# hzdr/PARIS

Measured on AMD Instinct MI355X. Metric: GVoxel-updates/s (voxels x projections / s), FDK hot path weight+filter+backproject, higher is better.
Workload: dtype f32

## Files before the change

include/paris_hip.h:

```cpp
#ifndef PARIS_HIP_H_
#define PARIS_HIP_H_

#include <stddef.h>
#include <stdint.h>

#ifdef __cplusplus
extern "C" {
#endif

#define PARIS_HIP_SUCCESS 0
#define PARIS_HIP_ERROR_INVALID_ARGUMENT 10001
#define PARIS_HIP_ERROR_NO_DEVICE 10002
#define PARIS_HIP_ERROR_UNSUPPORTED 10003

#define PARIS_HIP_CTX_DEFAULT 0u
#define PARIS_HIP_CTX_SYNCHRONOUS 1u
#define PARIS_HIP_CTX_LEGACY_STREAM 2u
#define PARIS_HIP_CTX_WARM 4u

typedef struct paris_detector_geometry {
    uint32_t n_row;
    uint32_t n_col;
    float l_px_row;
    float l_px_col;
// ... 194 lines not shown
                                uint32_t p_dim_y, uint32_t p_idx, float p_phi, float* d_v, uint32_t v_dim_x,
                                uint32_t v_dim_y, uint32_t v_dim_z, uint32_t v_offset,
                                const paris_detector_geometry* det_geo, const paris_volume_geometry* vol_geo,
                                int enable_angles, int enable_roi, const paris_region_of_interest* roi);

int paris_hip_forward_project(paris_hip_ctx* ctx, const float* d_v, uint32_t v_dim_x, uint32_t v_dim_y, uint32_t v_dim_z,
                              uint32_t v_offset, const paris_detector_geometry* det_geo, const paris_volume_geometry* vol_geo,
                              float* d_p, size_t p_pitch, size_t p_stride_bytes, uint32_t n_views, uint32_t p_dim_x,
                              uint32_t p_dim_y, const float* sin_phi, const float* cos_phi, float delta_s, float delta_t,
                              int accumulate);
int paris_hip_stage_forward_project(paris_hip_ctx* ctx, const float* d_v, uint32_t v_dim_x, uint32_t v_dim_y, uint32_t v_dim_z,
                                    uint32_t v_offset, const paris_detector_geometry* det_geo, const paris_volume_geometry* vol_geo,
                                    float* d_p, size_t p_pitch, uint32_t p_dim_x, uint32_t p_dim_y, uint32_t p_idx, float p_phi,
                                    int enable_angles, int accumulate);

const char* paris_hip_strerror(int status);
const char* paris_hip_version(void);
int paris_hip_has_experiments(void);
int paris_hip_last_backproject_ms(paris_hip_ctx* ctx, float* ms);
int paris_hip_backproject_timing_arm(paris_hip_ctx* ctx, uint32_t capacity);
int paris_hip_backproject_timing_collect(paris_hip_ctx* ctx, float* ms, uint32_t max_n, uint32_t* n_out);
int paris_hip_set_backproject_variant(paris_hip_ctx* ctx, int variant);
int paris_hip_set_backproject_tuning(paris_hip_ctx* ctx, int vx, int unroll, int tz, int lds_bytes);
int paris_hip_set_backproject_slice_shape(paris_hip_ctx* ctx, int waves, int row_groups);
int paris_hip_set_backproject_order(paris_hip_ctx* ctx, int order, int nontemporal);
int paris_hip_set_backproject_fast_division(paris_hip_ctx* ctx, int enable);
int paris_hip_set_backproject_vector_staging(paris_hip_ctx* ctx, int enable);
int paris_hip_fast_division_is_exact(paris_hip_ctx* ctx, float divisor, int* exact);
int paris_hip_lean_division_is_exact(paris_hip_ctx* ctx, float d_sd, float d_so, int* exact);
int paris_hip_lean_weighting_is_exact(paris_hip_ctx* ctx, float d_sd, float q_lo, float q_hi, int* exact);
int paris_hip_set_lean_validation(paris_hip_ctx* ctx, int enable);

#ifdef __cplusplus
}
#endif
#endif
```

paris_amd/_lib.py:

```python
import ctypes as C
import os

_HERE = os.path.dirname(os.path.abspath(__file__))
EXPERIMENTS_LIB_PATH = os.path.join(_HERE, "lib", "libparis_hip_experiments.so")
LIB_PATH = os.environ.get("PARIS_HIP_LIBRARY") or os.path.join(_HERE, "lib", "libparis_hip.so")

SUCCESS = 0
ERROR_INVALID_ARGUMENT = 10001
ERROR_NO_DEVICE = 10002
ERROR_UNSUPPORTED = 10003
CTX_DEFAULT = 0
CTX_SYNCHRONOUS = 1
CTX_LEGACY_STREAM = 2
CTX_WARM = 4
PIXEL_U8 = 1
PIXEL_U16 = 2
PIXEL_U32 = 3
PIXEL_F32 = 4


class DetectorGeometry(C.Structure):
    _fields_ = [("n_row", C.c_uint32), ("n_col", C.c_uint32),
                ("l_px_row", C.c_float), ("l_px_col", C.c_float),
                ("delta_s", C.c_float), ("delta_t", C.c_float),
# ... 115 lines not shown
    "paris_hip_short_scan_check": (C.c_int, [_P(DetectorGeometry), _P(ShortScan), _P(_f)]),
    "paris_hip_short_scan_weight_rows": (C.c_int, [_vp, _vp, _sz, _sz, _u32, _u32, _u32, _u32, _u32, _P(DetectorGeometry), _P(ShortScan),
                                                   _P(_f)]),
    "paris_hip_stage_short_scan_weight": (C.c_int, [_vp, _vp, _sz, _u32, _u32, _P(DetectorGeometry), _P(ShortScan), _u32, C.c_int,
                                                    _f]),
    "paris_hip_offset_detector_check": (C.c_int, [_P(DetectorGeometry), _P(_f)]),
    "paris_hip_offset_detector_weight_rows": (C.c_int, [_vp, _vp, _sz, _sz, _u32, _u32, _u32, _u32, _u32, _P(DetectorGeometry)]),
    "paris_hip_stage_offset_detector_weight": (C.c_int, [_vp, _vp, _sz, _u32, _u32, _P(DetectorGeometry)]),
    "paris_hip_stage_backproject": (C.c_int, [_vp, _vp, _sz, _u32, _u32, _u32, _f, _vp, _u32, _u32, _u32, _u32,
                                              _P(DetectorGeometry), _P(VolumeGeometry), C.c_int, C.c_int,
                                              _P(RegionOfInterest)]),
    "paris_hip_forward_project": (C.c_int, [_vp, _vp, _u32, _u32, _u32, _u32, _P(DetectorGeometry), _P(VolumeGeometry), _vp, _sz, _sz,
                                            _u32, _u32, _u32, _P(_f), _P(_f), _f, _f, C.c_int]),
    "paris_hip_stage_forward_project": (C.c_int, [_vp, _vp, _u32, _u32, _u32, _u32, _P(DetectorGeometry), _P(VolumeGeometry), _vp, _sz,
                                                  _u32, _u32, _u32, _f, C.c_int, C.c_int]),
    "paris_hip_strerror": (C.c_char_p, [C.c_int]),
    "paris_hip_version": (C.c_char_p, []),
    "paris_hip_last_backproject_ms": (C.c_int, [_vp, _P(_f)]),
    "paris_hip_backproject_timing_arm": (C.c_int, [_vp, _u32]),
    "paris_hip_backproject_timing_collect": (C.c_int, [_vp, _P(_f), _u32, _P(_u32)]),
    "paris_hip_set_backproject_variant": (C.c_int, [_vp, C.c_int]),
    "paris_hip_set_backproject_tuning": (C.c_int, [_vp, C.c_int, C.c_int, C.c_int, C.c_int]),
    "paris_hip_set_backproject_order": (C.c_int, [_vp, C.c_int, C.c_int]),
    "paris_hip_set_backproject_slice_shape": (C.c_int, [_vp, C.c_int, C.c_int]),
    "paris_hip_set_backproject_fast_division": (C.c_int, [_vp, C.c_int]),
    "paris_hip_set_backproject_vector_staging": (C.c_int, [_vp, C.c_int]),
    "paris_hip_fast_division_is_exact": (C.c_int, [_vp, _f, _P(C.c_int)]),
}

_lib = None


def load():
    global _lib
    if _lib is None:
        if not os.path.exists(LIB_PATH):
            raise ImportError(
                "paris_amd: %s not found -- build it with `python -c 'import __graft_entry__ as g; g.build()'` "
                "or `make -C paris_amd/csrc`; there is no CPU fallback" % LIB_PATH)
        if os.environ.get("PARIS_AMD_NO_TORCH") != "1":
            try:
                import torch
            except ImportError:
                pass
        lib = C.CDLL(LIB_PATH)
        for name, (res, args) in SIGNATURES.items():
# ... 23 lines not shown
```

paris_amd/backend.py:

```python
import ctypes as C

import numpy as np

from . import _lib
from ._lib import (DetectorGeometry, ParisHipError, RegionOfInterest, ShortScan, SubvolumeGeometry, SubvolumeInfo,
                   VolumeGeometry, check)

__all__ = ["DetectorGeometry", "VolumeGeometry", "SubvolumeGeometry", "RegionOfInterest", "SubvolumeInfo",
           "ParisHipError", "ShortScan", "Projection", "Volume", "FilterBuffer", "Backend", "get_devices", "set_device",
           "calculate_volume_geometry", "apply_roi", "filter_size", "load", "make_volume", "weight", "filter",
           "backproject", "forward_project", "short_scan_check", "offset_detector_check"]


class Projection:

    def __init__(self, buf, dim_x, dim_y, idx=0, phi=0.0, pitch=None, on_device=False, owner=None):
        self.buf = buf
        self.dim_x = dim_x
        self.dim_y = dim_y
        self.idx = idx
        self.phi = phi
        self.pitch = pitch if pitch is not None else dim_x * 4
        self.on_device = on_device
        self._owner = owner
# ... 332 lines not shown
              "paris_hip_forward_project")

    def last_backproject_ms(self):
        ms = C.c_float()
        check(self._L.paris_hip_last_backproject_ms(self._ctx, C.byref(ms)), "paris_hip_last_backproject_ms")
        return ms.value

    def backproject_timing_arm(self, capacity):
        check(self._L.paris_hip_backproject_timing_arm(self._ctx, capacity), "paris_hip_backproject_timing_arm")

    def backproject_timing_collect(self, max_n=65536):
        ms = (C.c_float * max_n)()
        n = C.c_uint32()
        check(self._L.paris_hip_backproject_timing_collect(self._ctx, ms, max_n, C.byref(n)),
              "paris_hip_backproject_timing_collect")
        return list(ms[:n.value])

    def set_backproject_variant(self, variant):
        check(self._L.paris_hip_set_backproject_variant(self._ctx, variant), "paris_hip_set_backproject_variant")

    def set_backproject_order(self, order=-1, nontemporal=-1):
        check(self._L.paris_hip_set_backproject_order(self._ctx, order, nontemporal), "paris_hip_set_backproject_order")

    def fast_division_is_exact(self, divisor):
        ok = C.c_int()
        check(self._L.paris_hip_fast_division_is_exact(self._ctx, divisor, C.byref(ok)), "paris_hip_fast_division_is_exact")
        return bool(ok.value)

    def set_backproject_vector_staging(self, enable=True):
        check(self._L.paris_hip_set_backproject_vector_staging(self._ctx, int(bool(enable))),
              "paris_hip_set_backproject_vector_staging")

    def set_backproject_fast_division(self, enable=True):
        check(self._L.paris_hip_set_backproject_fast_division(self._ctx, int(bool(enable))),
              "paris_hip_set_backproject_fast_division")

    def set_backproject_slice_shape(self, waves=0, row_groups=0):
        check(self._L.paris_hip_set_backproject_slice_shape(self._ctx, waves, row_groups),
              "paris_hip_set_backproject_slice_shape")

    def set_filter_window(self, window):
        check(self._L.paris_hip_set_filter_window(self._ctx, window), "paris_hip_set_filter_window")

    def set_filter_deferral(self, enable):
        check(self._L.paris_hip_set_filter_deferral(self._ctx, 2 if enable == 2 else int(bool(enable))), "paris_hip_set_filter_deferral")

# ... 165 lines not shown
```

paris_amd/csrc/backproject.hip:

```cpp
#include "bp_device.h"

#include <mutex>
#include <utility>

namespace
{
    __global__ void __launch_bounds__(256) fastdiv_validate_kernel(float c, float r, unsigned long long* mismatches)
    {
        const uint32_t t = blockIdx.x * 256u + threadIdx.x;
        unsigned int bad = 0;
        for(uint32_t i = 0; i < 256u; ++i)
        {
            const uint32_t bits = (i << 24) | t;
            const float x = __uint_as_float(bits);
            const float want = x / c - (1.f / 2.f);
            const float got = div_by_constant(x, c, r) - (1.f / 2.f);
            const bool same = __float_as_uint(want) == __float_as_uint(got);
            const bool both_nan = (want != want) && (got != got);
            const bool want_far = !(fabsf(want) <= 16777216.f);
            const bool got_far = !(fabsf(got) <= 16777216.f);
            if(!(same || both_nan || (want_far && got_far)))
                ++bad;
        }
        if(bad)
// ... 287 lines not shown
                       const paris_region_of_interest* roi, float sin_phi, float cos_phi, float delta_s, float delta_t,
                       BpParams& g, bool& fd, bool& skip)
{
    const size_t px = f16 ? sizeof(uint16_t) : sizeof(float);
    skip = false;
    if(int rc = paris_hip_bind(ctx))
        return rc;
    if(int rc = paris_hip_flush_pending_weight(ctx))
        return rc;
    if(d_p == nullptr || d_v == nullptr || det_geo == nullptr || vol_geo == nullptr || (enable_roi && roi == nullptr))
        return PARIS_HIP_ERROR_INVALID_ARGUMENT;
    if(p_dim_x == 0 || p_dim_y == 0 || p_pitch < static_cast<size_t>(p_dim_x) * px || p_pitch % px != 0)
        return PARIS_HIP_ERROR_INVALID_ARGUMENT;
    if(v_dim_x == 0 || v_dim_y == 0 || v_dim_z == 0)
    {
        skip = true;
        return PARIS_HIP_SUCCESS;
    }
    const uint64_t plane = static_cast<uint64_t>(v_dim_x) * v_dim_y;
    const uint32_t tz_auto = plane > (1ull << 20) ? (v_dim_z <= 256u ? 8u : TZ_DEFAULT) : (plane > (1ull << 18) ? 8u : TZ_DEFAULT);
    const uint32_t tz = ctx->bp_tz ? ctx->bp_tz : tz_auto;
    {
        const uint32_t tz_min = std::min(tz, 8u);
        const uint64_t ntx = (v_dim_x + 63u) / 64u, nty = (v_dim_y + 3u) / 4u, ntz = (v_dim_z + tz_min - 1u) / tz_min;
        const uint64_t zchunk = chunk_tiles(12u, tz_min, static_cast<uint32_t>(ntz), 64u);
        const uint64_t padded = std::max<uint64_t>(8ull * (8u * ((nty + 63u) / 64u)) * ntx * zchunk * ((ntz + zchunk - 1u) / zchunk),
                                                   8ull * ntx * nty * (ntz / 8u) + 8ull * 7u * 8u * ((nty + 63u) / 64u) * ntx);
        if(padded > 0x7fffff00ull)
            return PARIS_HIP_ERROR_UNSUPPORTED;
    }

    g = BpParams{};
    g.proj = d_p;
    g.proj_f16 = f16 ? 1u : 0u;
    g.vol = d_v;
    g.p_pitch = static_cast<uint32_t>(p_pitch / px);
    g.p_dim_x = p_dim_x;
    g.p_dim_y = p_dim_y;
    g.v_dim_x = v_dim_x;
    g.v_dim_y = v_dim_y;
    g.v_dim_z = v_dim_z;
    g.k_off = enable_roi ? roi->x1 : 0u;
    g.l_off = enable_roi ? roi->y1 : 0u;
    g.m_off = (enable_roi ? roi->z1 : 0u) + v_offset;
    g.x_base = centered_base(vol_geo->dim_x, vol_geo->l_vx_x);
    g.y_base = centered_base(vol_geo->dim_y, vol_geo->l_vx_y);
    g.z_base = centered_base(vol_geo->dim_z, vol_geo->l_vx_z);
    g.l_vx_x = vol_geo->l_vx_x;
    g.l_vx_y = vol_geo->l_vx_y;
    g.l_vx_z = vol_geo->l_vx_z;
// ... 18 lines not shown
        fd = fd && fd_x;
    }
    {
        const double x0 = g.x_base + static_cast<double>(g.k_off) * g.l_vx_x, x1 = g.x_base + (static_cast<double>(g.k_off) + v_dim_x - 1.0) * g.l_vx_x;
        const double y0 = g.y_base + static_cast<double>(g.l_off) * g.l_vx_y, y1 = g.y_base + (static_cast<double>(g.l_off) + v_dim_y - 1.0) * g.l_vx_y;
        const double reach = std::hypot(std::max(std::fabs(x0), std::fabs(x1)), std::max(std::fabs(y0), std::fabs(y1)));
        const double lo = std::ldexp(1.0, -40), hi = std::ldexp(1.0, 40);
        const bool ordinary = g.d_so >= lo && g.d_so <= hi && g.d_sd >= lo && g.d_sd <= hi;
        g.lean_div = (ctx->bp_lean_div != 0 && ordinary && std::isfinite(reach) && reach <= 0.9 * g.d_so) ? 1u : 0u;
        if(g.lean_div != 0u)
        {
            bool exact = false;
            if(int rc = paris_hip_lean_division_check(ctx, g.d_sd, g.d_so, &exact))
                return rc;
            g.lean_div = exact ? 1u : 0u;
        }
    }
    g.p_dim_x_f = static_cast<float>(p_dim_x);
    g.p_dim_y_f = static_cast<float>(p_dim_y);
    g.skip_invalid = (ctx->bp_skip_invalid != 0 && d_v != nullptr
                      && paris_hip_volume_is_clean(ctx, d_v, static_cast<size_t>(v_dim_x) * v_dim_y * v_dim_z * sizeof(float))) ? 1u : 0u;
    g.lds_floats = (ctx->bp_lds_bytes ? ctx->bp_lds_bytes : LDS_BYTES_DEFAULT) / sizeof(float);
    g.tz = tz;
    {
#ifdef PARIS_HIP_EXPERIMENTS
        static const int tile_nest = std::getenv("PARIS_TILE_NEST") ? std::atoi(std::getenv("PARIS_TILE_NEST")) : -1;
#else
        constexpr int tile_nest = -1;
#endif
        g.yfast = tile_nest >= 0 ? static_cast<uint32_t>(tile_nest) : (v_dim_z > 256u ? 2u : 0u);
    }
    g.order = ctx->bp_order >= 0 ? static_cast<uint32_t>(ctx->bp_order) : (plane > (1ull << 20) ? 15u : 18u);
    g.store_sc1 = volume_stream_policy(ctx, v_dim_x, v_dim_y, v_dim_z) == 2 ? 1u : 0u;
    g.stage_vec4 = (ctx->bp_stage_vec4 != 0 && g.p_pitch % 4u == 0 && reinterpret_cast<uintptr_t>(d_p) % (4u * px) == 0)
                       ? 1u : 0u;
    return PARIS_HIP_SUCCESS;
}

static int lane_width(const float* d_v, uint32_t v_dim_x)
{
    const uintptr_t addr = reinterpret_cast<uintptr_t>(d_v);
    if(v_dim_x % 4u == 0 && addr % 16u == 0)
        return 4;
    if(v_dim_x % 2u == 0 && addr % 8u == 0)
        return 2;
    return 1;
// ... 7 lines not shown
{
    BpParams g;
    bool fd = false, skip = false;
    if(int rc = fill_params(ctx, d_p, f16, p_pitch, p_dim_x, p_dim_y, d_v, v_dim_x, v_dim_y, v_dim_z, v_offset, det_geo, vol_geo,
                            enable_roi, roi, sin_phi, cos_phi, delta_s, delta_t, g, fd, skip))
        return rc;
    if(skip)
        return paris_hip_finish(ctx);

    const bool timed = !ctx->bp_start.empty();
    const size_t ev = timed ? static_cast<size_t>(ctx->bp_launches % ctx->bp_start.size()) : 0u;
    if(timed)
        PARIS_HIP_TRY(hipEventRecord(ctx->bp_start[ev], ctx->stream));
    if(ctx->bp_variant == 4 && !f16)
    {
        FusedParams fp{};
        fp.g = g;
        fp.n_proj = 1;
        fp.proj_tab[0] = d_p;
        fp.sin_phi[0] = sin_phi;
        fp.cos_phi[0] = cos_phi;
        const int width = lane_width(d_v, v_dim_x);
        const int vx = ctx->bp_vx == 4 && width == 4 ? 4 : (ctx->bp_vx == 1 || width < 2 ? 1 : 2);
        paris_hip_bp_launch_fused(&fp, vx, ctx->bp_tz == 8u ? 8 : (ctx->bp_tz == 32u ? 32 : 16), volume_stream_policy(ctx, v_dim_x, v_dim_y, v_dim_z) != 0, fd, ctx->stream);
    }
    else
    if(ctx->bp_variant == 1)
    {
        const dim3 grid((v_dim_x + 255u) / 256u, v_dim_y, v_dim_z);
        if(v_dim_y > 65535u || v_dim_z > 65535u)
            return PARIS_HIP_ERROR_UNSUPPORTED;
        hipLaunchKernelGGL(bp_gather_kernel, grid, dim3(256), 0, ctx->stream, g);
    }
    else
    {
        int vx = lane_width(d_v, v_dim_x);
        if(ctx->bp_vx && ctx->bp_vx < vx)
            vx = ctx->bp_vx;
        if(ctx->bp_vx == 0 && vx == 4 && ctx->bp_variant != 3 && ctx->bp_variant != 5)
        {
            const uint64_t tiles = static_cast<uint64_t>((v_dim_x + 63u) / 64u) * ((v_dim_y + 15u) / 16u) * ((v_dim_z + g.tz - 1u) / g.tz);
            if(tiles < 2048u)
                vx = 2;
        }
        const bool deep_big = g.tz == 16u && ctx->bp_tz == 0u && static_cast<uint64_t>(v_dim_x) * v_dim_y > (1ull << 20);
        if(deep_big && ctx->bp_unroll == 0 && ctx->bp_lds_bytes == 0u && vx == 4)
            g.lds_floats = 40u * 1024u / sizeof(float);
// ... 558 lines not shown
{
    if(int rc = paris_hip_flush_deferred(ctx))
        return rc;
    return batch_impl(ctx, d_p, true, p_pitch, p_stride_bytes, n_proj, p_dim_x, p_dim_y, d_v, v_dim_x, v_dim_y, v_dim_z, v_offset, det_geo,
                      vol_geo, enable_roi, roi, sin_phi, cos_phi, delta_s, delta_t);
}

static int batch_impl(paris_hip_ctx* ctx, const void* d_p, bool f16, size_t p_pitch, size_t p_stride_bytes, uint32_t n_proj, uint32_t p_dim_x,
                      uint32_t p_dim_y, float* d_v, uint32_t v_dim_x, uint32_t v_dim_y, uint32_t v_dim_z, uint32_t v_offset,
                      const paris_detector_geometry* det_geo, const paris_volume_geometry* vol_geo, int enable_roi,
                      const paris_region_of_interest* roi, const float* sin_phi, const float* cos_phi, float delta_s, float delta_t,
                      const void* const* ptrs)
{
    const size_t px = f16 ? sizeof(uint16_t) : sizeof(float);
    if(ctx == nullptr || sin_phi == nullptr || cos_phi == nullptr || (ptrs == nullptr && p_stride_bytes % px != 0))
        return PARIS_HIP_ERROR_INVALID_ARGUMENT;
    if(n_proj == 0)
        return paris_hip_finish(ctx);
    if(ptrs == nullptr && n_proj > 1 && p_stride_bytes < p_pitch * static_cast<size_t>(p_dim_y))
        return PARIS_HIP_ERROR_INVALID_ARGUMENT;
    const auto where = [&](uint32_t i) { return ptrs != nullptr ? static_cast<const char*>(ptrs[i]) : static_cast<const char*>(d_p) + static_cast<size_t>(i) * p_stride_bytes; };

    const int width = d_v != nullptr ? lane_width(d_v, v_dim_x) : 1;
    bool deep_box_fits = true;
    {
        const double d_so = std::fabs(static_cast<double>(det_geo->d_so)), d_sd = d_so + std::fabs(static_cast<double>(det_geo->d_od));
        const double mag = d_so > 0.0 ? d_sd / d_so : 1.0;
        const double rows = 32.0 * vol_geo->l_vx_z * mag / det_geo->l_px_col + 4.0 * std::max(vol_geo->l_vx_x, vol_geo->l_vx_y) * mag / det_geo->l_px_col + 8.0;
        const double cols = 64.0 * std::max(vol_geo->l_vx_x, vol_geo->l_vx_y) * mag / det_geo->l_px_row + 16.0;
        const double budget = ctx->bp_lds_bytes != 0u ? ctx->bp_lds_bytes : 32.0 * 1024.0;
        deep_box_fits = std::isfinite(rows) && std::isfinite(cols) && rows * std::max(132.0, cols) * sizeof(float) <= budget;
    }
    int fused_vx = ((v_dim_z <= 16u || !deep_box_fits) && width >= 2) ? 2 : 1;
    if(ctx->bp_vx == 4 && width == 4)
        fused_vx = 4;
    else if(ctx->bp_vx == 2 && width >= 2)
        fused_vx = 2;
    else if(ctx->bp_vx == 1)
        fused_vx = 1;
    int fused_tz = fused_vx == 1 ? ((v_dim_z <= 16u || !deep_box_fits) ? 16 : 32) : 16;
    if(ctx->bp_tz == 8u && fused_vx != 1)
        fused_tz = 8;
    else if(ctx->bp_tz == 16u)
        fused_tz = 16;
    else if(ctx->bp_tz == 32u && fused_vx == 1)
        fused_tz = 32;
    const bool fused_ok = n_proj > 1 && (ctx->bp_variant == 0 || ctx->bp_variant == 4) && d_v != nullptr;
    if(!fused_ok)
    {
        const unsigned saved = ctx->flags;
        ctx->flags &= ~PARIS_HIP_CTX_SYNCHRONOUS;
        int rc = PARIS_HIP_SUCCESS;
        for(uint32_t i = 0; i < n_proj && rc == PARIS_HIP_SUCCESS; ++i)
        {
            const char* p = where(i);
            rc = backproject_impl(ctx, p, f16, p_pitch, p_dim_x, p_dim_y, d_v, v_dim_x, v_dim_y, v_dim_z, v_offset, det_geo, vol_geo,
                                  enable_roi, roi, sin_phi[i], cos_phi[i], delta_s, delta_t);
        }
        ctx->flags = saved;
        if(rc != PARIS_HIP_SUCCESS)
            return rc;
        return paris_hip_finish(ctx);
    }

    const bool nt = volume_stream_policy(ctx, v_dim_x, v_dim_y, v_dim_z) != 0;
    for(uint32_t first = 0; first < n_proj; first += FUSED_MAX)
    {
        const uint32_t n = std::min<uint32_t>(FUSED_MAX, n_proj - first);
        FusedParams fp{};
        bool fd = false, skip = false;
        const char* p0 = where(first);
        if(int rc = fill_params(ctx, p0, f16, p_pitch, p_dim_x, p_dim_y, d_v, v_dim_x, v_dim_y, v_dim_z, v_offset, det_geo,
                                vol_geo, enable_roi, roi, sin_phi[first], cos_phi[first], delta_s, delta_t, fp.g, fd, skip))
            return rc;
        if(skip)
            break;
        fp.n_proj = n;
        if(ctx->bp_order < 0 && fp.g.order == 15u)
            fp.g.order = fused_vx == 1 ? 17u : (fused_vx == 2 ? 16u : 15u);
#ifdef PARIS_HIP_EXPERIMENTS
        static const bool x_fast = std::getenv("PARIS_FUSED_XFAST") != nullptr;
#else
        constexpr bool x_fast = false;
#endif
        fp.g.yfast = x_fast ? 0u : 1u;
        if(ctx->bp_lds_bytes == 0u)
            fp.g.lds_floats = 32u * 1024u / sizeof(float);
        for(uint32_t i = 0; i < n; ++i)
        {
            fp.sin_phi[i] = sin_phi[first + i];
            fp.cos_phi[i] = cos_phi[first + i];
            fp.proj_tab[i] = where(first + i);
            if(reinterpret_cast<uintptr_t>(fp.proj_tab[i]) % (4u * px) != 0)
                fp.g.stage_vec4 = 0u;
        }
        for(uint32_t i = n; i < FUSED_MAX; ++i)
            fp.proj_tab[i] = fp.proj_tab[0];
        const bool timed = !ctx->bp_start.empty();
        const size_t ev = timed ? static_cast<size_t>(ctx->bp_launches % ctx->bp_start.size()) : 0u;
        if(timed)
            PARIS_HIP_TRY(hipEventRecord(ctx->bp_start[ev], ctx->stream));
        paris_hip_bp_launch_fused(&fp, fused_vx, fused_tz, nt, fd, ctx->stream);
        if(timed)
            PARIS_HIP_TRY(hipEventRecord(ctx->bp_stop[ev], ctx->stream));
        ++ctx->bp_launches;
        for(uint32_t i = 0; i < n && !ctx->upload_targets.empty(); ++i)
            if(int rc = paris_hip_note_projection_use(ctx, where(first + i), p_pitch * p_dim_y))
                return rc;
    }
    return paris_hip_finish(ctx);
}

extern "C" int paris_hip_last_backproject_ms(paris_hip_ctx* ctx, float* ms)
{
    if(int rc = paris_hip_flush_deferred(ctx))
        return rc;
    if(ctx == nullptr || ms == nullptr || ctx->bp_launches == 0 || ctx->bp_start.empty())
        return PARIS_HIP_ERROR_INVALID_ARGUMENT;
    if(int rc = paris_hip_bind(ctx))
        return rc;
    const size_t ev = static_cast<size_t>((ctx->bp_launches - 1) % ctx->bp_start.size());
    PARIS_HIP_TRY(hipEventSynchronize(ctx->bp_stop[ev]));
    PARIS_HIP_TRY(hipEventElapsedTime(ms, ctx->bp_start[ev], ctx->bp_stop[ev]));
    return PARIS_HIP_SUCCESS;
}

extern "C" int paris_hip_set_backproject_variant(paris_hip_ctx* ctx, int variant)
{
    if(int rc = paris_hip_flush_deferred(ctx))
        return rc;
    if(ctx == nullptr || variant < 0 || variant > 5)
        return PARIS_HIP_ERROR_INVALID_ARGUMENT;
#ifndef PARIS_HIP_EXPERIMENTS
    if(variant == 3 || variant == 5)
        return PARIS_HIP_ERROR_UNSUPPORTED;
#endif
    ctx->bp_variant = variant;
    return PARIS_HIP_SUCCESS;
}

extern "C" int paris_hip_set_backproject_order(paris_hip_ctx* ctx, int order, int nontemporal)
{
    if(int rc = paris_hip_flush_deferred(ctx))
        return rc;
    if(ctx == nullptr || !(order == -1 || order == 0 || order == 1 || order == 5 || order == 8 || order == 9 || order == 12 || (order >= 14 && order <= 18)) || nontemporal < -1 || nontemporal > 2)
        return PARIS_HIP_ERROR_INVALID_ARGUMENT;
// ... 107 lines not shown
```

paris_amd/csrc/backproject_fused.hip:

```cpp
#define PARIS_BP_SINGLE_INSTRUCTION_FLOOR 1
#if (defined(PARIS_TIMING_ONLY_NO_BARRIERS) || defined(PARIS_TIMING_ONLY_STAGE_ONCE)) && !defined(PARIS_HIP_EXPERIMENTS)
#error "the timing-only switches compute WRONG results: they exist in the experiments build only (make EXPERIMENTS=1)"
#endif
#include "bp_device.h"

namespace
{
#ifndef PARIS_FUSED_PIPELINE
#define PARIS_FUSED_PIPELINE 1
#endif
#ifndef PARIS_FUSED_WAVES
#define PARIS_FUSED_WAVES 3
#endif
    constexpr int FIXED_STRIDE = 132;

    template <int VX, int TZ, bool NT, bool FD>
    __global__ void __launch_bounds__(256, PARIS_FUSED_WAVES + (VX == 2 ? 1 : VX == 1 ? (TZ == 32 ? 1 : 4) : 0) + (TZ == 8 ? 1 : 0)) bp_fused_kernel(const FusedParams fp)
    {
        extern __shared__ __attribute__((aligned(16))) float lds[];
        BpParams g = fp.g;
        using vec = typename vec_of<VX>::type;
        constexpr uint32_t XL = 64u / VX;
        constexpr uint32_t RW = VX;
        constexpr uint32_t TY = 4u * RW;

        const uint32_t tid = threadIdx.x;
        const uint32_t lane = tid & 63u;
        const uint32_t wave = tid >> 6;

        uint32_t bx, by, bz;
        if(!tile_of_block(g, blockIdx.x, bx, by, bz))
            return;
        const uint32_t k0 = bx * 64u;
        const uint32_t l0 = by * TY;
        const uint32_t m0 = bz * TZ;
        const uint32_t k1 = min(k0 + 63u, g.v_dim_x - 1u);
        const uint32_t l1 = min(l0 + TY - 1u, g.v_dim_y - 1u);
        const uint32_t m1 = min(m0 + TZ - 1u, g.v_dim_z - 1u);
        const uint32_t mcount = m1 - m0 + 1u;

        const uint32_t xq = lane % XL, yy = lane / XL;
        const uint32_t k = k0 + xq * VX;
        const uint32_t l = l0 + wave * RW + yy;
        const bool active = k < g.v_dim_x && l < g.v_dim_y;

        const size_t slice = static_cast<size_t>(g.v_dim_x) * g.v_dim_y;
        float* vp = g.vol + (static_cast<size_t>(m0) * g.v_dim_y + l) * g.v_dim_x + k;
        vec acc[TZ] = {};
#pragma unroll
        for(int z = 0; z < TZ; ++z)
            if(active && static_cast<uint32_t>(z) < mcount)
                acc[z] = load_voxels<VX, NT>(vp + z * slice);

        const float z_first = g.z_base + static_cast<float>(g.m_off + m0) * g.l_vx_z;
        const float z_last = g.z_base + static_cast<float>(g.m_off + m1) * g.l_vx_z;
        __shared__ int box_tab[FUSED_MAX * BOX_WORDS];
        if(wave * 16u < fp.n_proj)
            tile_boxes_to_lds(g, fp.sin_phi, fp.cos_phi, wave * 16u, fp.n_proj, k0, k1, l0, l1, m0, m1, lane, g.lds_floats, FIXED_STRIDE, box_tab);
        for(uint32_t p = 0; p < fp.n_proj; ++p)
// ... 73 lines not shown
                if(g.skip_invalid != 0u && __all(all_none ? 1 : 0) != 0)
                {
                }
                else if(wave_inside && fixed)
                    add_projection(std::true_type{}, std::true_type{}, std::true_type{}, the_stride{});
                else if(wave_inside)
                    add_projection(std::true_type{}, std::true_type{}, std::true_type{}, no_stride{});
                else if(all_fast && mcount == TZ && fixed)
                    add_projection(std::true_type{}, std::true_type{}, std::false_type{}, the_stride{});
                else if(all_fast && mcount == TZ)
                    add_projection(std::true_type{}, std::true_type{}, std::false_type{}, no_stride{});
                else if(all_fast)
                    add_projection(std::true_type{}, std::false_type{}, std::false_type{}, no_stride{});
                else
                    add_projection(std::false_type{}, std::false_type{}, std::false_type{}, no_stride{});
            }
        }
#pragma unroll
        for(int z = 0; z < TZ; ++z)
            if(active && static_cast<uint32_t>(z) < mcount)
                store_voxels<VX, NT>(vp + z * slice, acc[z], g.store_sc1 != 0u);
    }

    template <int VX, int TZ, bool NT, bool FD>
    void launch_fused(FusedParams& fp, hipStream_t stream)
    {
        BpParams& g = fp.g;
        g.tz = TZ;
        g.ntx = (g.v_dim_x + 63u) / 64u;
        g.nty = (g.v_dim_y + 4u * VX - 1u) / (4u * VX);
        g.ntz = (g.v_dim_z + TZ - 1u) / TZ;
        settle_order(g);
        g.zchunk = chunk_tiles(g.order, TZ, g.ntz, 32u);
        const uint32_t blocks = static_cast<uint32_t>(grid_blocks(g));
        hipLaunchKernelGGL((bp_fused_kernel<VX, TZ, NT, FD>), dim3(blocks), dim3(256), g.lds_floats * sizeof(float), stream, fp);
    }

    template <int VX, int TZ>
    void launch_fused_flags(FusedParams& fp, bool nt, bool fd, hipStream_t stream)
    {
        if(nt && fd)
            launch_fused<VX, TZ, true, true>(fp, stream);
        else if(nt)
            launch_fused<VX, TZ, true, false>(fp, stream);
        else if(fd)
            launch_fused<VX, TZ, false, true>(fp, stream);
        else
            launch_fused<VX, TZ, false, false>(fp, stream);
    }
}

void paris_hip_bp_launch_fused(const void* fused_params, int vx, int tz, bool nt, bool fd, hipStream_t stream)
{
    FusedParams fp = *static_cast<const FusedParams*>(fused_params);
    if(vx == 1 && tz == 32)
        launch_fused_flags<1, 32>(fp, nt, fd, stream);
    else if(vx == 1)
        launch_fused_flags<1, 16>(fp, nt, fd, stream);
    else if(vx == 2 && tz == 8)
        launch_fused_flags<2, 8>(fp, nt, fd, stream);
    else if(vx == 2)
        launch_fused_flags<2, 16>(fp, nt, fd, stream);
    else if(tz == 8)
        launch_fused_flags<4, 8>(fp, nt, fd, stream);
    else
        launch_fused_flags<4, 16>(fp, nt, fd, stream);
}

void paris_hip_warm_backproject_fused()
{
    hipFuncAttributes a{};
    (void)hipFuncGetAttributes(&a, reinterpret_cast<const void*>((&bp_fused_kernel<1, 32, true, true>)));
}
```

paris_amd/csrc/bp_device.h:

```cpp
#ifndef PARIS_HIP_BP_DEVICE_H_
#define PARIS_HIP_BP_DEVICE_H_

#include "paris_hip_internal.h"
#include "ieee_lean.h"

#include <algorithm>
#include <cmath>
#include <cstdlib>
#include <cstring>
#include <type_traits>

#ifndef PARIS_BP_SINGLE_INSTRUCTION_FLOOR
#define PARIS_BP_SINGLE_INSTRUCTION_FLOOR 0
#endif

namespace
{
    struct BpParams
    {
        const void* proj;
        uint32_t proj_f16;
        float* vol;
        uint32_t p_pitch;
        uint32_t p_dim_x, p_dim_y;
        uint32_t v_dim_x, v_dim_y, v_dim_z;
        uint32_t k_off, l_off, m_off;
        float x_base, y_base, z_base;
        float l_vx_x, l_vx_y, l_vx_z;
        float sin_phi, cos_phi;
        float d_so, d_sd;
        float min_h, min_v;
        float l_px_x, l_px_y;
        float rcp_l_px_y;
        float rcp_l_px_x;
        float p_dim_x_f, p_dim_y_f;
        uint32_t lds_floats;
        uint32_t tz;
        uint32_t ntx, nty, ntz;
        uint32_t order;
        uint32_t zchunk;
        uint32_t lean_div;
        const float* colstate;
        uint32_t store_sc1;
        uint32_t stage_vec4;
        uint32_t skip_invalid;
        uint32_t yfast;
    };

    struct ColConst
    {
        float factor, h, u;
    };

    __device__ __forceinline__ float div_by_constant(float x, float c, float r)
    {
        const float q = x * r;
        const float e = __builtin_fmaf(-q, c, x);
        return __builtin_fmaf(e, r, q);
    }

    template <bool FD>
    __device__ __forceinline__ ColConst column_constants(const BpParams& g, uint32_t K, uint32_t L)
    {
        const float x_k = g.x_base + static_cast<float>(K) * g.l_vx_x;
        const float y_l = g.y_base + static_cast<float>(L) * g.l_vx_y;
        const float s = x_k * g.cos_phi + y_l * g.sin_phi;
        const float t = -x_k * g.sin_phi + y_l * g.cos_phi;
        const float den = s + g.d_so;
        ColConst c;
// ... 31 lines not shown
    }

    template <int VX> struct vec_of;
    template <> struct vec_of<1> { using type = float; };
    template <> struct vec_of<2> { using type = float2; };
    template <> struct vec_of<4> { using type = float4; };

    template <int VX> __device__ __forceinline__ float& elem(typename vec_of<VX>::type& v, int j);
    template <> __device__ __forceinline__ float& elem<1>(float& v, int) { return v; }
    template <> __device__ __forceinline__ float& elem<2>(float2& v, int j) { return j == 0 ? v.x : v.y; }
    template <> __device__ __forceinline__ float& elem<4>(float4& v, int j)
    {
        return j == 0 ? v.x : (j == 1 ? v.y : (j == 2 ? v.z : v.w));
    }

    __host__ __device__ inline uint32_t dealt_band(uint32_t nty, uint32_t order)
    {
        const uint32_t grp = 1u << (order - 14u);
        return grp * ((nty + 8u * grp - 1u) / (8u * grp));
    }

    __host__ __device__ inline uint32_t order18_tail_group_log2(const BpParams& g)
    {
        return g.yfast == 1u ? 3u : 1u;
    }

    inline uint64_t grid_blocks(const BpParams& g)
    {
        const uint64_t total = static_cast<uint64_t>(g.ntx) * g.nty * g.ntz;
        if(g.order == 5u)
            return ((total + 7u) / 8u) * 8u;
#ifdef PARIS_HIP_EXPERIMENTS
        if(g.order == 8u || g.order == 9u)
            return 8ull * ((g.nty + 7u) / 8u) * g.ntx * g.ntz;
        if(g.order == 12u)
            return 8ull * ((g.nty + 7u) / 8u) * g.ntx * g.zchunk * ((g.ntz + g.zchunk - 1u) / g.zchunk);
#endif
        if(g.order == 18u)
            return 8ull * (static_cast<uint64_t>(g.ntx) * g.nty * (g.ntz / 8u)
                           + static_cast<uint64_t>(g.ntz % 8u) * dealt_band(g.nty, 14u + order18_tail_group_log2(g)) * g.ntx);
        if(g.order >= 14u && g.order <= 17u)
            return 8ull * dealt_band(g.nty, g.order) * g.ntx * g.zchunk * ((g.ntz + g.zchunk - 1u) / g.zchunk);
        return total;
    }

    inline void settle_order(BpParams& g)
    {
// ... 629 lines not shown
    __device__ __forceinline__ float finish_tap(const Column& col, const Tap& t)
    {
        const float interp_y1 = col.wx2 * t.q11 + col.wx1 * t.q21;
        const float interp_y2 = col.wx2 * t.q12 + col.wx1 * t.q22;
        const float wy2 = 1.f - t.wy1;
        float det = wy2 * interp_y1 + t.wy1 * interp_y2;
        if(!ALLVALID)
            det = t.valid ? det : 0.f;
        return 0.5f * det * col.u * col.u;
    }

    constexpr int FUSED_MAX = 64;

    struct FusedParams
    {
        BpParams g;
        uint32_t n_proj;
        float sin_phi[FUSED_MAX];
        float cos_phi[FUSED_MAX];
        const void* proj_tab[FUSED_MAX];
    };
}

void paris_hip_bp_launch_fused(const void* fused_params, int vx, int tz, bool nt, bool fd, hipStream_t stream);

#endif
```

paris_amd/csrc/paris_hip_internal.h:

```cpp
#ifndef PARIS_HIP_INTERNAL_H_
#define PARIS_HIP_INTERNAL_H_

#include <hip/hip_runtime.h>

#include <cstddef>
#include <array>
#include <cstdint>
#include <map>
#include <vector>

#include "paris_hip.h"

#pragma clang fp contract(off)

#define PARIS_HIP_TRY(expr)                                   \
    do                                                        \
    {                                                         \
        hipError_t paris_hip_err__ = (expr);                  \
        if(paris_hip_err__ != hipSuccess)                     \
            return static_cast<int>(paris_hip_err__);         \
    } while(0)

struct paris_hip_fft_plan
{
    float2* d_twiddle = nullptr;
    float2* d_tab_first = nullptr;
    float2* d_tab_mid[3] = {nullptr, nullptr, nullptr};
};

struct paris_hip_filter_info
{
    uint32_t size = 0;
    float* d_kp = nullptr;
};

struct paris_hip_ctx
{
    int device = 0;
    hipStream_t stream = nullptr;
    bool owns_stream = false;
    unsigned flags = 0;
    std::vector<hipEvent_t> bp_start, bp_stop;
    uint64_t bp_launches = 0;
    int bp_variant = 0;
    int bp_vx = 0, bp_unroll = 0;
    uint32_t bp_tz = 0, bp_lds_bytes = 0;
    int bp_order = -1;
    int bp_slice_nw = 0, bp_slice_rpl = 0;
    int bp_nt = -1;
    int bp_stage_vec4 = 1;
    int bp_fastdiv = 1;
    int bp_skip_invalid = 1;
    std::map<uintptr_t, size_t> clean_volumes;
    std::map<uintptr_t, size_t> volume_allocs;
    int bp_lean_div = 1;
    std::map<uint32_t, bool> fastdiv_exact;
    std::map<std::array<uint32_t, 4>, bool> lean_checks;
    int lean_validate = 1;
    bool filter_lds_attr_set = false;
    bool filter_r16_attr_set[5] = {false, false, false, false, false};
    int filter_variant = 0;
    std::map<uint32_t, paris_hip_fft_plan> plans;
    std::map<const float*, paris_hip_filter_info> filters;
    int stage_fusion = 0;
    struct pending_weight_t
    {
        bool active = false;
        float* d_p = nullptr;
        size_t pitch = 0;
        uint32_t dim_x = 0, dim_y = 0, row_first = 0, row_count = 0;
// ... 224 lines not shown
```

Baseline: 782.3.

## Pick fused backprojection tile footprint per projection batch from angles

Adds narrower x-tile footprints (32 and 16 lanes wide, taller in y) to the fused backprojection kernel. The host picks, per projection batch, the footprint whose projected detector box is smallest and fits the LDS budget, using the mean |sin| and |cos| of the batch angles. The aim is to shrink the staged detector region and let more batches use the deep single-voxel path. In exchange it adds more kernel template instantiations, a more complex grid order mapping, and host-side angle scanning per batch.

```diff
diff --git a/include/paris_hip.h b/include/paris_hip.h
--- a/include/paris_hip.h
+++ b/include/paris_hip.h
@@ -240,6 +240,8 @@
 int paris_hip_backproject_timing_collect(paris_hip_ctx* ctx, float* ms, uint32_t max_n, uint32_t* n_out);
 int paris_hip_set_backproject_variant(paris_hip_ctx* ctx, int variant);
 int paris_hip_set_backproject_tuning(paris_hip_ctx* ctx, int vx, int unroll, int tz, int lds_bytes);
+int paris_hip_set_fused_footprint(paris_hip_ctx* ctx, int lanes_x);
+int paris_hip_last_fused_shape(paris_hip_ctx* ctx, int* lanes_x, int* vx, int* tz);
 int paris_hip_set_backproject_slice_shape(paris_hip_ctx* ctx, int waves, int row_groups);
 int paris_hip_set_backproject_order(paris_hip_ctx* ctx, int order, int nontemporal);
 int paris_hip_set_backproject_fast_division(paris_hip_ctx* ctx, int enable);
diff --git a/paris_amd/_lib.py b/paris_amd/_lib.py
--- a/paris_amd/_lib.py
+++ b/paris_amd/_lib.py
@@ -161,6 +161,8 @@
     "paris_hip_set_backproject_variant": (C.c_int, [_vp, C.c_int]),
     "paris_hip_set_backproject_tuning": (C.c_int, [_vp, C.c_int, C.c_int, C.c_int, C.c_int]),
     "paris_hip_set_backproject_order": (C.c_int, [_vp, C.c_int, C.c_int]),
+    "paris_hip_set_fused_footprint": (C.c_int, [_vp, C.c_int]),
+    "paris_hip_last_fused_shape": (C.c_int, [_vp, _P(C.c_int), _P(C.c_int), _P(C.c_int)]),
     "paris_hip_set_backproject_slice_shape": (C.c_int, [_vp, C.c_int, C.c_int]),
     "paris_hip_set_backproject_fast_division": (C.c_int, [_vp, C.c_int]),
     "paris_hip_set_backproject_vector_staging": (C.c_int, [_vp, C.c_int]),
diff --git a/paris_amd/backend.py b/paris_amd/backend.py
--- a/paris_amd/backend.py
+++ b/paris_amd/backend.py
@@ -378,6 +378,14 @@
     def set_backproject_order(self, order=-1, nontemporal=-1):
         check(self._L.paris_hip_set_backproject_order(self._ctx, order, nontemporal), "paris_hip_set_backproject_order")
 
+    def set_fused_footprint(self, lanes_x=0):
+        check(self._L.paris_hip_set_fused_footprint(self._ctx, lanes_x), "paris_hip_set_fused_footprint")
+
+    def last_fused_shape(self):
+        lanes_x, vx, tz = C.c_int(), C.c_int(), C.c_int()
+        check(self._L.paris_hip_last_fused_shape(self._ctx, C.byref(lanes_x), C.byref(vx), C.byref(tz)), "paris_hip_last_fused_shape")
+        return lanes_x.value, vx.value, tz.value
+
     def fast_division_is_exact(self, divisor):
         ok = C.c_int()
         check(self._L.paris_hip_fast_division_is_exact(self._ctx, divisor, C.byref(ok)), "paris_hip_fast_division_is_exact")
diff --git a/paris_amd/csrc/backproject.hip b/paris_amd/csrc/backproject.hip
--- a/paris_amd/csrc/backproject.hip
+++ b/paris_amd/csrc/backproject.hip
@@ -333,10 +333,17 @@
     const uint32_t tz = ctx->bp_tz ? ctx->bp_tz : tz_auto;
     {
         const uint32_t tz_min = std::min(tz, 8u);
-        const uint64_t ntx = (v_dim_x + 63u) / 64u, nty = (v_dim_y + 3u) / 4u, ntz = (v_dim_z + tz_min - 1u) / tz_min;
+        const uint64_t ntz = (v_dim_z + tz_min - 1u) / tz_min;
         const uint64_t zchunk = chunk_tiles(12u, tz_min, static_cast<uint32_t>(ntz), 64u);
-        const uint64_t padded = std::max<uint64_t>(8ull * (8u * ((nty + 63u) / 64u)) * ntx * zchunk * ((ntz + zchunk - 1u) / zchunk),
-                                                   8ull * ntx * nty * (ntz / 8u) + 8ull * 7u * 8u * ((nty + 63u) / 64u) * ntx);
+        uint64_t padded = 0;
+        for(uint32_t w = 64u; w >= 16u; w /= 2u)
+        {
+            const uint32_t h = 256u / w;
+            const uint64_t ntx = (static_cast<uint64_t>(v_dim_x) + w - 1u) / w, nty = (static_cast<uint64_t>(v_dim_y) + h - 1u) / h;
+            padded = std::max<uint64_t>({padded,
+                                         8ull * (8u * ((nty + 63u) / 64u)) * ntx * zchunk * ((ntz + zchunk - 1u) / zchunk),
+                                         8ull * ntx * nty * (ntz / 8u) + 8ull * 7u * 8u * ((nty + 63u) / 64u) * ntx});
+        }
         if(padded > 0x7fffff00ull)
             return PARIS_HIP_ERROR_UNSUPPORTED;
     }
@@ -401,6 +408,8 @@
                       && paris_hip_volume_is_clean(ctx, d_v, static_cast<size_t>(v_dim_x) * v_dim_y * v_dim_z * sizeof(float))) ? 1u : 0u;
     g.lds_floats = (ctx->bp_lds_bytes ? ctx->bp_lds_bytes : LDS_BYTES_DEFAULT) / sizeof(float);
     g.tz = tz;
+    g.tile_w = 64u;
+    g.tile_h = 16u;
     {
 #ifdef PARIS_HIP_EXPERIMENTS
         static const int tile_nest = std::getenv("PARIS_TILE_NEST") ? std::atoi(std::getenv("PARIS_TILE_NEST")) : -1;
@@ -454,7 +463,7 @@
         fp.cos_phi[0] = cos_phi;
         const int width = lane_width(d_v, v_dim_x);
         const int vx = ctx->bp_vx == 4 && width == 4 ? 4 : (ctx->bp_vx == 1 || width < 2 ? 1 : 2);
-        paris_hip_bp_launch_fused(&fp, vx, ctx->bp_tz == 8u ? 8 : (ctx->bp_tz == 32u ? 32 : 16), volume_stream_policy(ctx, v_dim_x, v_dim_y, v_dim_z) != 0, fd, ctx->stream);
+        paris_hip_bp_launch_fused(&fp, vx, ctx->bp_tz == 8u ? 8 : (ctx->bp_tz == 32u ? 32 : 16), 64, volume_stream_policy(ctx, v_dim_x, v_dim_y, v_dim_z) != 0, fd, ctx->stream);
     }
     else
     if(ctx->bp_variant == 1)
@@ -1059,29 +1068,66 @@
     const auto where = [&](uint32_t i) { return ptrs != nullptr ? static_cast<const char*>(ptrs[i]) : static_cast<const char*>(d_p) + static_cast<size_t>(i) * p_stride_bytes; };
 
     const int width = d_v != nullptr ? lane_width(d_v, v_dim_x) : 1;
-    bool deep_box_fits = true;
+    const double fp_budget = ctx->bp_lds_bytes != 0u ? ctx->bp_lds_bytes : 32.0 * 1024.0;
+    double fp_rows, fp_px_per_vx;
     {
         const double d_so = std::fabs(static_cast<double>(det_geo->d_so)), d_sd = d_so + std::fabs(static_cast<double>(det_geo->d_od));
         const double mag = d_so > 0.0 ? d_sd / d_so : 1.0;
-        const double rows = 32.0 * vol_geo->l_vx_z * mag / det_geo->l_px_col + 4.0 * std::max(vol_geo->l_vx_x, vol_geo->l_vx_y) * mag / det_geo->l_px_col + 8.0;
-        const double cols = 64.0 * std::max(vol_geo->l_vx_x, vol_geo->l_vx_y) * mag / det_geo->l_px_row + 16.0;
-        const double budget = ctx->bp_lds_bytes != 0u ? ctx->bp_lds_bytes : 32.0 * 1024.0;
-        deep_box_fits = std::isfinite(rows) && std::isfinite(cols) && rows * std::max(132.0, cols) * sizeof(float) <= budget;
-    }
-    int fused_vx = ((v_dim_z <= 16u || !deep_box_fits) && width >= 2) ? 2 : 1;
-    if(ctx->bp_vx == 4 && width == 4)
-        fused_vx = 4;
-    else if(ctx->bp_vx == 2 && width >= 2)
-        fused_vx = 2;
-    else if(ctx->bp_vx == 1)
-        fused_vx = 1;
-    int fused_tz = fused_vx == 1 ? ((v_dim_z <= 16u || !deep_box_fits) ? 16 : 32) : 16;
-    if(ctx->bp_tz == 8u && fused_vx != 1)
-        fused_tz = 8;
-    else if(ctx->bp_tz == 16u)
-        fused_tz = 16;
-    else if(ctx->bp_tz == 32u && fused_vx == 1)
-        fused_tz = 32;
+        fp_rows = 32.0 * vol_geo->l_vx_z * mag / det_geo->l_px_col + 4.0 * std::max(vol_geo->l_vx_x, vol_geo->l_vx_y) * mag / det_geo->l_px_col + 8.0;
+        fp_px_per_vx = std::max(vol_geo->l_vx_x, vol_geo->l_vx_y) * mag / det_geo->l_px_row;
+    }
+    const auto box_cols = [&](int w, uint32_t first, uint32_t n) {
+        double s = 0.0, c = 0.0;
+        for(uint32_t i = 0; i < n; ++i)
+        {
+            s += std::fabs(static_cast<double>(sin_phi[first + i]));
+            c += std::fabs(static_cast<double>(cos_phi[first + i]));
+        }
+        return (w * s / n + (256 / w) * c / n) * fp_px_per_vx + 16.0;
+    };
+    const auto box_fits = [&](int w, double cols) {
+        const double stride = w == 64 ? std::max(132.0, cols) : cols + 8.0;
+        return std::isfinite(fp_rows) && std::isfinite(cols) && fp_rows * stride * sizeof(float) <= fp_budget;
+    };
+    const auto fused_shape = [&](uint32_t first, uint32_t n, int& fused_vx, int& fused_tz, int& lanes_x) {
+        bool deep_box_fits = false;
+        lanes_x = 64;
+        if(ctx->bp_fused_footprint != 0)
+        {
+            lanes_x = ctx->bp_fused_footprint;
+            deep_box_fits = true;
+        }
+        else
+        {
+            double best = 0.0;
+            for(int w = 64; w >= 16; w /= 2)
+            {
+                const double cols = box_cols(w, first, n);
+                if(box_fits(w, cols) && (!deep_box_fits || cols < best))
+                {
+                    deep_box_fits = true;
+                    best = cols;
+                    lanes_x = w;
+                }
+            }
+        }
+        fused_vx = ((v_dim_z <= 16u || !deep_box_fits) && width >= 2 && ctx->bp_fused_footprint == 0) ? 2 : 1;
+        if(ctx->bp_vx == 4 && width == 4)
+            fused_vx = 4;
+        else if(ctx->bp_vx == 2 && width >= 2)
+            fused_vx = 2;
+        else if(ctx->bp_vx == 1)
+            fused_vx = 1;
+        fused_tz = fused_vx == 1 ? ((v_dim_z <= 16u || !deep_box_fits) ? 16 : 32) : 16;
+        if(ctx->bp_tz == 8u && fused_vx != 1)
+            fused_tz = 8;
+        else if(ctx->bp_tz == 16u)
+            fused_tz = 16;
+        else if(ctx->bp_tz == 32u && fused_vx == 1)
+            fused_tz = 32;
+        if(fused_vx != 1)
+            lanes_x = 64;
+    };
     const bool fused_ok = n_proj > 1 && (ctx->bp_variant == 0 || ctx->bp_variant == 4) && d_v != nullptr;
     if(!fused_ok)
     {
@@ -1113,8 +1159,13 @@
         if(skip)
             break;
         fp.n_proj = n;
+        int fused_vx, fused_tz, lanes_x;
+        fused_shape(first, n, fused_vx, fused_tz, lanes_x);
         if(ctx->bp_order < 0 && fp.g.order == 15u)
-            fp.g.order = fused_vx == 1 ? 17u : (fused_vx == 2 ? 16u : 15u);
+        {
+            const int tile_h = 256 * fused_vx / lanes_x;
+            fp.g.order = tile_h == 4 ? 17u : (tile_h == 8 ? 16u : 15u);
+        }
 #ifdef PARIS_HIP_EXPERIMENTS
         static const bool x_fast = std::getenv("PARIS_FUSED_XFAST") != nullptr;
 #else
@@ -1137,7 +1188,10 @@
         const size_t ev = timed ? static_cast<size_t>(ctx->bp_launches % ctx->bp_start.size()) : 0u;
         if(timed)
             PARIS_HIP_TRY(hipEventRecord(ctx->bp_start[ev], ctx->stream));
-        paris_hip_bp_launch_fused(&fp, fused_vx, fused_tz, nt, fd, ctx->stream);
+        paris_hip_bp_launch_fused(&fp, fused_vx, fused_tz, lanes_x, nt, fd, ctx->stream);
+        ctx->last_fused_lanes_x = lanes_x / fused_vx;
+        ctx->last_fused_vx = fused_vx;
+        ctx->last_fused_tz = fused_tz;
         if(timed)
             PARIS_HIP_TRY(hipEventRecord(ctx->bp_stop[ev], ctx->stream));
         ++ctx->bp_launches;
@@ -1159,6 +1213,28 @@
     const size_t ev = static_cast<size_t>((ctx->bp_launches - 1) % ctx->bp_start.size());
     PARIS_HIP_TRY(hipEventSynchronize(ctx->bp_stop[ev]));
     PARIS_HIP_TRY(hipEventElapsedTime(ms, ctx->bp_start[ev], ctx->bp_stop[ev]));
+    return PARIS_HIP_SUCCESS;
+}
+
+extern "C" int paris_hip_set_fused_footprint(paris_hip_ctx* ctx, int lanes_x)
+{
+    if(int rc = paris_hip_flush_deferred(ctx))
+        return rc;
+    if(ctx == nullptr || !(lanes_x == 0 || lanes_x == 64 || lanes_x == 32 || lanes_x == 16))
+        return PARIS_HIP_ERROR_INVALID_ARGUMENT;
+    ctx->bp_fused_footprint = lanes_x;
+    return PARIS_HIP_SUCCESS;
+}
+
+extern "C" int paris_hip_last_fused_shape(paris_hip_ctx* ctx, int* lanes_x, int* vx, int* tz)
+{
+    if(int rc = paris_hip_flush_deferred(ctx))
+        return rc;
+    if(ctx == nullptr || lanes_x == nullptr || vx == nullptr || tz == nullptr || ctx->last_fused_vx == 0)
+        return PARIS_HIP_ERROR_INVALID_ARGUMENT;
+    *lanes_x = ctx->last_fused_lanes_x;
+    *vx = ctx->last_fused_vx;
+    *tz = ctx->last_fused_tz;
     return PARIS_HIP_SUCCESS;
 }
 
diff --git a/paris_amd/csrc/backproject_fused.hip b/paris_amd/csrc/backproject_fused.hip
--- a/paris_amd/csrc/backproject_fused.hip
+++ b/paris_amd/csrc/backproject_fused.hip
@@ -14,14 +14,15 @@
 #endif
     constexpr int FIXED_STRIDE = 132;
 
-    template <int VX, int TZ, bool NT, bool FD>
+    template <int VX, int TZ, bool NT, bool FD, int TW = 64>
     __global__ void __launch_bounds__(256, PARIS_FUSED_WAVES + (VX == 2 ? 1 : VX == 1 ? (TZ == 32 ? 1 : 4) : 0) + (TZ == 8 ? 1 : 0)) bp_fused_kernel(const FusedParams fp)
     {
+        static_assert(TW == 64 || (VX == 1 && (TW == 32 || TW == 16)), "narrow footprints are built for one voxel per lane only");
         extern __shared__ __attribute__((aligned(16))) float lds[];
         BpParams g = fp.g;
         using vec = typename vec_of<VX>::type;
-        constexpr uint32_t XL = 64u / VX;
-        constexpr uint32_t RW = VX;
+        constexpr uint32_t XL = static_cast<uint32_t>(TW) / VX;
+        constexpr uint32_t RW = 64u / XL;
         constexpr uint32_t TY = 4u * RW;
 
         const uint32_t tid = threadIdx.x;
@@ -31,10 +32,10 @@
         uint32_t bx, by, bz;
         if(!tile_of_block(g, blockIdx.x, bx, by, bz))
             return;
-        const uint32_t k0 = bx * 64u;
+        const uint32_t k0 = bx * static_cast<uint32_t>(TW);
         const uint32_t l0 = by * TY;
         const uint32_t m0 = bz * TZ;
-        const uint32_t k1 = min(k0 + 63u, g.v_dim_x - 1u);
+        const uint32_t k1 = min(k0 + static_cast<uint32_t>(TW) - 1u, g.v_dim_x - 1u);
         const uint32_t l1 = min(l0 + TY - 1u, g.v_dim_y - 1u);
         const uint32_t m1 = min(m0 + TZ - 1u, g.v_dim_z - 1u);
         const uint32_t mcount = m1 - m0 + 1u;
@@ -154,38 +155,48 @@
                 store_voxels<VX, NT>(vp + z * slice, acc[z], g.store_sc1 != 0u);
     }
 
-    template <int VX, int TZ, bool NT, bool FD>
+    template <int VX, int TZ, bool NT, bool FD, int TW>
     void launch_fused(FusedParams& fp, hipStream_t stream)
     {
         BpParams& g = fp.g;
         g.tz = TZ;
-        g.ntx = (g.v_dim_x + 63u) / 64u;
-        g.nty = (g.v_dim_y + 4u * VX - 1u) / (4u * VX);
+        g.tile_w = TW;
+        g.tile_h = 256u * VX / TW;
+        g.ntx = (g.v_dim_x + g.tile_w - 1u) / g.tile_w;
+        g.nty = (g.v_dim_y + g.tile_h - 1u) / g.tile_h;
         g.ntz = (g.v_dim_z + TZ - 1u) / TZ;
         settle_order(g);
         g.zchunk = chunk_tiles(g.order, TZ, g.ntz, 32u);
         const uint32_t blocks = static_cast<uint32_t>(grid_blocks(g));
-        hipLaunchKernelGGL((bp_fused_kernel<VX, TZ, NT, FD>), dim3(blocks), dim3(256), g.lds_floats * sizeof(float), stream, fp);
+        hipLaunchKernelGGL((bp_fused_kernel<VX, TZ, NT, FD, TW>), dim3(blocks), dim3(256), g.lds_floats * sizeof(float), stream, fp);
     }
 
-    template <int VX, int TZ>
+    template <int VX, int TZ, int TW = 64>
     void launch_fused_flags(FusedParams& fp, bool nt, bool fd, hipStream_t stream)
     {
         if(nt && fd)
-            launch_fused<VX, TZ, true, true>(fp, stream);
+            launch_fused<VX, TZ, true, true, TW>(fp, stream);
         else if(nt)
-            launch_fused<VX, TZ, true, false>(fp, stream);
+            launch_fused<VX, TZ, true, false, TW>(fp, stream);
         else if(fd)
-            launch_fused<VX, TZ, false, true>(fp, stream);
+            launch_fused<VX, TZ, false, true, TW>(fp, stream);
         else
-            launch_fused<VX, TZ, false, false>(fp, stream);
+            launch_fused<VX, TZ, false, false, TW>(fp, stream);
     }
 }
 
-void paris_hip_bp_launch_fused(const void* fused_params, int vx, int tz, bool nt, bool fd, hipStream_t stream)
+void paris_hip_bp_launch_fused(const void* fused_params, int vx, int tz, int tile_w, bool nt, bool fd, hipStream_t stream)
 {
     FusedParams fp = *static_cast<const FusedParams*>(fused_params);
-    if(vx == 1 && tz == 32)
+    if(vx == 1 && tz == 32 && tile_w == 16)
+        launch_fused_flags<1, 32, 16>(fp, nt, fd, stream);
+    else if(vx == 1 && tz == 32 && tile_w == 32)
+        launch_fused_flags<1, 32, 32>(fp, nt, fd, stream);
+    else if(vx == 1 && tile_w == 16)
+        launch_fused_flags<1, 16, 16>(fp, nt, fd, stream);
+    else if(vx == 1 && tile_w == 32)
+        launch_fused_flags<1, 16, 32>(fp, nt, fd, stream);
+    else if(vx == 1 && tz == 32)
         launch_fused_flags<1, 32>(fp, nt, fd, stream);
     else if(vx == 1)
         launch_fused_flags<1, 16>(fp, nt, fd, stream);
diff --git a/paris_amd/csrc/bp_device.h b/paris_amd/csrc/bp_device.h
--- a/paris_amd/csrc/bp_device.h
+++ b/paris_amd/csrc/bp_device.h
@@ -45,6 +45,7 @@
         uint32_t stage_vec4;
         uint32_t skip_invalid;
         uint32_t yfast;
+        uint32_t tile_w, tile_h;
     };
 
     struct ColConst
@@ -122,7 +123,9 @@
 
     __host__ __device__ inline uint32_t order18_tail_group_log2(const BpParams& g)
     {
-        return g.yfast == 1u ? 3u : 1u;
+        if(g.yfast != 1u)
+            return 1u;
+        return g.tile_w == 32u ? 2u : (g.tile_w == 16u ? 1u : 3u);
     }
 
     inline uint64_t grid_blocks(const BpParams& g)
@@ -798,6 +801,6 @@
     };
 }
 
-void paris_hip_bp_launch_fused(const void* fused_params, int vx, int tz, bool nt, bool fd, hipStream_t stream);
+void paris_hip_bp_launch_fused(const void* fused_params, int vx, int tz, int tile_w, bool nt, bool fd, hipStream_t stream);
 
 #endif
diff --git a/paris_amd/csrc/paris_hip_internal.h b/paris_amd/csrc/paris_hip_internal.h
--- a/paris_amd/csrc/paris_hip_internal.h
+++ b/paris_amd/csrc/paris_hip_internal.h
@@ -46,6 +46,8 @@
     int bp_vx = 0, bp_unroll = 0;
     uint32_t bp_tz = 0, bp_lds_bytes = 0;
     int bp_order = -1;
+    int bp_fused_footprint = 0;
+    int last_fused_lanes_x = 0, last_fused_vx = 0, last_fused_tz = 0;
     int bp_slice_nw = 0, bp_slice_rpl = 0;
     int bp_nt = -1;
     int bp_stage_vec4 = 1;
```

Measured after the change: 781.3. No clear change (-0.1%).
